# RookieJunChen/FullSubNet-plus

Hardware: AMD Instinct MI355X
Metric: STFT frames/sec (257-bin, 2 s clips), FullSubNet+ forward (higher is better)
Workload: dtype f32

## Files before the change

fullsubnet_plus_amd/csrc/lstm.hip:

```cpp
#include <cstring>

#include "fsnp_common.h"
#include "lstm_common.h"

namespace fsnp {

template <int EX>
__host__ __device__ __forceinline__ int e_frag_index(int e, int k) {
    return ((((k >> 3) * 2) + (k & 1)) * EX + e) * 4 + ((k >> 1) & 3);
}

struct WStream {
    __amdgpu_buffer_rsrc_t rsrc;
    int voff;
};
template <int NT>
__device__ __forceinline__ float4 wload(const WStream& ws, int g, int n) {
    const auto v = __builtin_amdgcn_raw_buffer_load_b128(ws.rsrc, ws.voff, (g * NT + n) * 1024, 0);
    return __builtin_bit_cast(float4, v);
}

template <int NT, int EX>
__device__ __forceinline__ void mfma_groups(f32x16 (&acc)[NT], float (&accx)[EX > 0 ? EX : 1][NT], float4 (&b)[NT],
                                            const float4* __restrict__ A, const float4* __restrict__ AE, int ngroups,
                                            const WStream& ws, int& gnext, int groups_total) {
    float4 a = A[0];
    float4 ae[EX > 0 ? EX : 1];
#pragma unroll
    for (int e = 0; e < EX; ++e) ae[e] = AE[e];
    for (int g = 0; g < ngroups; ++g) {
        const int gn = (g + 1 < ngroups ? g + 1 : g);
        const float4 an = A[gn * 64];
        float4 aen[EX > 0 ? EX : 1];
#pragma unroll
        for (int e = 0; e < EX; ++e) aen[e] = AE[gn * 2 * EX + e];
        if constexpr (EX == 0) {
#pragma unroll
            for (int n = 0; n < NT; ++n) {
                acc[n] = __builtin_amdgcn_mfma_f32_32x32x2f32(a.x, b[n].x, acc[n], 0, 0, 0);
                acc[n] = __builtin_amdgcn_mfma_f32_32x32x2f32(a.y, b[n].y, acc[n], 0, 0, 0);
                acc[n] = __builtin_amdgcn_mfma_f32_32x32x2f32(a.z, b[n].z, acc[n], 0, 0, 0);
                acc[n] = __builtin_amdgcn_mfma_f32_32x32x2f32(a.w, b[n].w, acc[n], 0, 0, 0);
                b[n] = wload<NT>(ws, gnext, n);
                __builtin_amdgcn_sched_barrier(0);
            }
        } else {
            constexpr int HALF = NT / 2;
#pragma unroll
            for (int hb = 0; hb < NT; hb += HALF) {
#pragma unroll
                for (int n = hb; n < hb + HALF; ++n) {
                    acc[n] = __builtin_amdgcn_mfma_f32_32x32x2f32(a.x, b[n].x, acc[n], 0, 0, 0);
                    acc[n] = __builtin_amdgcn_mfma_f32_32x32x2f32(a.y, b[n].y, acc[n], 0, 0, 0);
                    acc[n] = __builtin_amdgcn_mfma_f32_32x32x2f32(a.z, b[n].z, acc[n], 0, 0, 0);
                    acc[n] = __builtin_amdgcn_mfma_f32_32x32x2f32(a.w, b[n].w, acc[n], 0, 0, 0);
                }
                __builtin_amdgcn_sched_barrier(0);
#pragma unroll
                for (int n = hb; n < hb + HALF; ++n)
#pragma unroll
                    for (int e = 0; e < EX; ++e) {
                        float v = accx[e][n];
                        v = fmaf(ae[e].x, b[n].x, v);
                        v = fmaf(ae[e].y, b[n].y, v);
                        v = fmaf(ae[e].z, b[n].z, v);
                        accx[e][n] = fmaf(ae[e].w, b[n].w, v);
                    }
                __builtin_amdgcn_sched_barrier(0);
#pragma unroll
                for (int n = hb; n < hb + HALF; ++n) b[n] = wload<NT>(ws, gnext, n);
                __builtin_amdgcn_sched_barrier(0);
            }
        }
        gnext = (gnext + 1 == groups_total) ? 0 : gnext + 1;
        a = an;
#pragma unroll
        for (int e = 0; e < EX; ++e) ae[e] = aen[e];
    }
}

__device__ __forceinline__ unsigned short bf16_bits(float v) {
    const unsigned u = __float_as_uint(v);
    return (unsigned short)((u + 0x7FFFu + ((u >> 16) & 1u)) >> 16);
}
__host__ __device__ __forceinline__ int a_frag_index_bf16(int row, int k) {
    return (((k >> 4) * 64) + (((k >> 3) & 1) * 32) + row) * 8 + (k & 7);
}

template <int ST, int UW, int HBLO = 0>
__device__ __forceinline__ void lstm_cell(f32x16 (&acc)[4 * ST], f32x2 (&c)[ST][8], float* __restrict__ Hs, int wave,
                                          int lane, unsigned short* __restrict__ Hb = nullptr) {
#pragma unroll
    for (int s = 0; s < ST; ++s) {
        const int k = wave * UW + s * 32 + (lane & 31);
        const int kbase = (((k >> 3) * 64) + ((k & 1) * 32)) * 4 + ((k >> 1) & 3);
#pragma unroll
        for (int r = 0; r < 16; r += 2) {
            auto rd = [](float v) {
                if constexpr (ST > 1) { float o; asm("v_accvgpr_read_b32 %0, %1" : "=v"(o) : "a"(v)); return o; }
                else return v;
            };
            const f32x2 h = lstm_cell_pair(f32x2{rd(acc[s][r]), rd(acc[s][r + 1])}, f32x2{rd(acc[ST + s][r]), rd(acc[ST + s][r + 1])},
                                           f32x2{rd(acc[2 * ST + s][r]), rd(acc[2 * ST + s][r + 1])},
                                           f32x2{rd(acc[3 * ST + s][r]), rd(acc[3 * ST + s][r + 1])}, c[s][r >> 1]);
            const int row = (r & 3) + 8 * (r >> 2) + 4 * (lane >> 5);
            Hs[kbase + row * 4] = h.x;
            Hs[kbase + (row + 1) * 4] = h.y;
            if (Hb) {
                const unsigned short hx = bf16_bits(h.x), hy = bf16_bits(h.y);
                Hb[a_frag_index_bf16(row, k)] = hx; Hb[a_frag_index_bf16(row + 1, k)] = hy;
                if constexpr (HBLO > 0) {
                    Hb[HBLO + a_frag_index_bf16(row, k)] = bf16_bits(h.x - __uint_as_float((unsigned)hx << 16));
                    Hb[HBLO + a_frag_index_bf16(row + 1, k)] = bf16_bits(h.y - __uint_as_float((unsigned)hy << 16));
                }
            }
        }
    }
}

using bf16x8 = __attribute__((ext_vector_type(8))) __bf16;
template <int NT, int EX, int ALO>
__device__ __forceinline__ void mfma_groups_bf16(f32x16 (&acc)[NT], float (&accx)[EX > 0 ? EX : 1][NT], float4 (&b)[NT],
                                                 const float4* __restrict__ A, const float4* __restrict__ AE, int nsteps,
                                                 const WStream& ws, int& gnext, int groups_total, int lane) {
    float4 a = A[0], al = A[ALO];
    for (int g = 0; g < nsteps; ++g) {
        const float4 an = A[(g + 1 < nsteps ? g + 1 : g) * 64], aln = A[ALO + (g + 1 < nsteps ? g + 1 : g) * 64];
        float4 he[EX > 0 ? EX : 1][2];
        if constexpr (EX > 0) {
            const int kg = 2 * g + (lane >> 5);
#pragma unroll
            for (int e = 0; e < EX; ++e) { he[e][0] = AE[(kg * 2 + 0) * EX + e]; he[e][1] = AE[(kg * 2 + 1) * EX + e]; }
        }
#pragma unroll
        for (int n = 0; n < NT; ++n) {
            if constexpr (EX > 0) {
                const unsigned w0 = __float_as_uint(b[n].x), w1 = __float_as_uint(b[n].y), w2 = __float_as_uint(b[n].z),
                               w3 = __float_as_uint(b[n].w);
#pragma unroll
                for (int e = 0; e < EX; ++e) {
                    float v = accx[e][n];
                    v = fmaf(he[e][0].x, __uint_as_float(w0 << 16), v);
                    v = fmaf(he[e][1].x, __uint_as_float(w0 & 0xFFFF0000u), v);
                    v = fmaf(he[e][0].y, __uint_as_float(w1 << 16), v);
                    v = fmaf(he[e][1].y, __uint_as_float(w1 & 0xFFFF0000u), v);
                    v = fmaf(he[e][0].z, __uint_as_float(w2 << 16), v);
                    v = fmaf(he[e][1].z, __uint_as_float(w2 & 0xFFFF0000u), v);
                    v = fmaf(he[e][0].w, __uint_as_float(w3 << 16), v);
                    accx[e][n] = fmaf(he[e][1].w, __uint_as_float(w3 & 0xFFFF0000u), v);
                }
            }
            acc[n] = __builtin_amdgcn_mfma_f32_32x32x16_bf16(__builtin_bit_cast(bf16x8, a), __builtin_bit_cast(bf16x8, b[n]),
                                                             acc[n], 0, 0, 0);
            if constexpr (ALO > 0)
                acc[n] = __builtin_amdgcn_mfma_f32_32x32x16_bf16(__builtin_bit_cast(bf16x8, al), __builtin_bit_cast(bf16x8, b[n]),
                                                                 acc[n], 0, 0, 0);
            b[n] = wload<NT>(ws, gnext, n);
            __builtin_amdgcn_sched_barrier(0);
        }
        gnext = (gnext + 1 == groups_total) ? 0 : gnext + 1;
        a = an; al = aln;
    }
}

template <int ST, int UW, int EX, int NT>
__device__ __forceinline__ void lstm_cell_extra(float (&accx)[EX > 0 ? EX : 1][NT], float (&cx)[EX > 0 ? EX : 1][ST],
                                                const float* __restrict__ bias, float* __restrict__ He, int wave,
                                                int lane) {
#pragma unroll
    for (int e = 0; e < EX; ++e)
#pragma unroll
        for (int s = 0; s < ST; ++s) {
            float g4[4];
#pragma unroll
            for (int q = 0; q < 4; ++q) {
                const float v = accx[e][q * ST + s];
                g4[q] = v + __shfl_xor(v, 32) + (bias ? bias[(q * ST + s) * 32] : 0.0f);
            }
            const float cn = fast_sigmoid(g4[1]) * cx[e][s] + fast_sigmoid(g4[0]) * fast_tanh(g4[2]);
            cx[e][s] = cn;
            const float h = fast_sigmoid(g4[3]) * fast_tanh(cn);
            if (lane < 32) He[e_frag_index<EX>(e, wave * UW + s * 32 + lane)] = h;
        }
}

template <int HID, int KX, int OUT, int EX, bool PROF, int NW, bool BF>
__global__ __launch_bounds__(64 * NW) __attribute__((amdgpu_waves_per_eu(NW / 4, NW / 4)))
void lstm2_fc_kernel(LstmWeights w, LstmArgs a) {
    static_assert(OUT == 2, "FC lane mapping assumes output_size == 2");
    static_assert(EX >= 0 && EX <= 4, "at most 4 VALU rows per tile (one FC wave per extra row)");
    static_assert(NW % 4 == 0 && NW >= 4, "whole waves per SIMD");
    constexpr int NTHR = 64 * NW;
    constexpr int UW = HID / NW, ST = UW / 32, NT = 4 * ST;
    static_assert(UW % 32 == 0 && UW * NW == HID, "hidden/NW must be a multiple of 32");
    constexpr int KGX = KX / 8, KGH = HID / 8, KG0 = KGX + KGH;
    constexpr int KSB = HID / 16;
    constexpr int KG1 = BF ? KGH + KSB : 2 * KGH, KGT = KG0 + KG1;
    static_assert(KGH % 4 == 0, "FC k-split");
    static_assert(!BF || HID % 16 == 0, "bf16 k-steps");
    constexpr int RT = 32 + EX;
    constexpr int EXA = EX > 0 ? EX : 1;

    extern __shared__ __attribute__((aligned(16))) unsigned char smem_raw[];
    float4* Xs = reinterpret_cast<float4*>(smem_raw);
    float4* H0s = Xs + KGX * 64;
    float4* H1s = H0s + KGH * 64;
    float4* XEs = H1s + KGH * 64;
    float4* HE0s = XEs + KGX * 2 * EX;
    float4* HE1s = HE0s + KGH * 2 * EX;
    float4* Wfc4 = HE1s + KGH * 2 * EX;
    RowDesc* rows_s = reinterpret_cast<RowDesc*>(Wfc4 + OUT * KGH * 2);
    constexpr int BL = BF ? 1 : 2;
    constexpr bool HILO = BF && EX == 0;
    float* Bs = reinterpret_cast<float*>(rows_s + RT);
    float4* H0b = reinterpret_cast<float4*>(Bs + BL * NW * NT * 32);

    const int tid = threadIdx.x;
    const int lane = tid & 63;
    const int wave = __builtin_amdgcn_readfirstlane(tid >> 6);
    const int slot0 = blockIdx.x * RT;
    const int Tp = a.Tp;

    __shared__ unsigned long long clk_s[2];
    if (a.clk != nullptr && tid == 0) {
        clk_s[1] = __builtin_amdgcn_s_memrealtime();
        clk_s[0] = __builtin_amdgcn_s_memtime();
        if (blockIdx.x == 0) { a.clk[0] = clk_s[0]; a.clk[1] = clk_s[1]; a.clk[4] = 0ull; a.clk[5] = 0ull; a.clk[6] = ~0ull; }
    }

    for (int i = tid; i < (KGX + 2 * KGH) * (64 + 2 * EX); i += NTHR) Xs[i] = make_float4(0.f, 0.f, 0.f, 0.f);
    for (int i = tid; i < OUT * KGH * 2; i += NTHR) {
        const int o = i / (KGH * 2), kg = (i >> 1) % KGH, kh = i & 1;
        const float* wr = w.wfc + (size_t)o * HID + kg * 8 + kh;
        Wfc4[i] = make_float4(wr[0], wr[2], wr[4], wr[6]);
    }
    if (tid < RT) rows_s[tid] = a.rows[slot0 + tid];
    for (int i = tid; i < BL * NW * NT * 32; i += NTHR) {
        const int col = i & 31, n = (i >> 5) % NT, wv = (i / (32 * NT)) % NW, layer = BF ? 1 : i / (32 * NT * NW);
        Bs[i] = w.bias[layer * 4 * HID + (n / ST) * HID + wv * UW + (n % ST) * 32 + col];
    }
    __syncthreads();
    if constexpr (BF) {
        if (tid < 32) reinterpret_cast<float*>(Xs)[a_frag_index(tid, w.NIN)] = 1.0f;
        if (EX > 0 && tid < EX) reinterpret_cast<float*>(XEs)[e_frag_index<EXA>(tid, w.NIN)] = 1.0f;
    }

    const bool dense = a.dense != nullptr;
    const float* __restrict__ gbase = dense ? a.dense : a.att_mag;
    const int gstep = dense ? w.NIN : a.FP;
    auto plan = [&](const RowDesc& rd, int j) -> int {
        if (!rd.valid || j >= w.NIN) return -1;
        if (dense) return rd.b * Tp * w.NIN + j;
        return sb_feature_offset(j, rd.f, rd.b * Tp * a.FP, a.F, a.NSBN, a.NFBN, a.fb_rel, a.fb_branch_stride);
    };
    auto row_md = [&](const RowDesc& rd, int slot, NormMD& md, const NormMD*& md_row) {
        md.m = 0.0f; md.d = 1.0f; md_row = nullptr;
        if (dense || !rd.valid) return;
        if (a.md_row != nullptr) md_row = a.md_row + (size_t)slot * Tp;
        else md = a.md_utt[rd.b];
    };
    constexpr int JSTEP = NTHR / 32, NG = (KX + JSTEP - 1) / JSTEP;
    const int grow = tid & 31;
    int goff[NG], xdst[NG];
    NormMD md; const NormMD* md_row;
    {
        const RowDesc rd = rows_s[grow];
#pragma unroll
        for (int i = 0; i < NG; ++i) {
            const int j = (tid >> 5) + JSTEP * i;
            goff[i] = (j < KX && !(BF && j == w.NIN)) ? plan(rd, j) : -2;
            xdst[i] = a_frag_index(grow, j < KX ? j : 0);
        }
        row_md(rd, slot0 + grow, md, md_row);
    }
    int goffx = -1, xdstx = 0;
    NormMD mdx = {0.0f, 1.0f}; const NormMD* mdx_row = nullptr;
    bool havex = EX > 0 && tid < EX * KX;
    if (BF && havex && tid % KX == w.NIN) havex = false;
    if (havex) {
        const int e = tid / KX, j = tid % KX;
        const RowDesc rd = rows_s[32 + e];
        goffx = plan(rd, j);
        xdstx = e_frag_index<EXA>(e, j);
        row_md(rd, slot0 + 32 + e, mdx, mdx_row);
    }

    float* Xf = reinterpret_cast<float*>(Xs);
    float* XEf = reinterpret_cast<float*>(XEs);
    {
        const NormMD m0 = md_row ? md_row[0] : md;
#pragma unroll
        for (int i = 0; i < NG; ++i)
            if (goff[i] != -2) Xf[xdst[i]] = goff[i] >= 0 ? (gbase[goff[i]] - m0.m) / m0.d : 0.0f;
        if (havex) {
            const NormMD mx = mdx_row ? mdx_row[0] : mdx;
            XEf[xdstx] = goffx >= 0 ? (gbase[goffx] - mx.m) / mx.d : 0.0f;
        }
    }

    const float* __restrict__ bias_l0 = BF ? nullptr : Bs + ((0 * NW + wave) * NT) * 32 + (lane & 31);
    const float* __restrict__ bias_l1 = Bs + (((BL - 1) * NW + wave) * NT) * 32 + (lane & 31);
    f32x2 c0[ST][8], c1[ST][8];
    float cx0[EXA][ST], cx1[EXA][ST];
#pragma unroll
    for (int s = 0; s < ST; ++s) {
#pragma unroll
        for (int r = 0; r < 8; ++r) { c0[s][r] = f32x2{0.0f, 0.0f}; c1[s][r] = f32x2{0.0f, 0.0f}; }
#pragma unroll
        for (int e = 0; e < EXA; ++e) { cx0[e][s] = 0.0f; cx1[e][s] = 0.0f; }
    }

    WStream ws;
    ws.rsrc = __builtin_amdgcn_make_buffer_rsrc(const_cast<float*>(w.wpack) + (size_t)wave * KGT * NT * 256, 0,
                                                KGT * NT * 1024, 0x00020000);
    ws.voff = lane * 16;
    float4 breg[NT];
#pragma unroll
    for (int n = 0; n < NT; ++n) breg[n] = wload<NT>(ws, 0, n);
    int gnext = 1;
    auto run_groups = [&](f32x16 (&acc_)[NT], float (&accx_)[EXA][NT], const float4* A_, const float4* AE_, int ng) {
        mfma_groups<NT, EX>(acc_, accx_, breg, A_, AE_, ng, ws, gnext, KGT);
    };

    const int fc_row = (wave & 3) * 8 + (lane & 7);
    const int fc_o = (lane >> 3) & 1;
    const int fc_kp = lane >> 4;
    const RowDesc fc_rd = rows_s[fc_row];
    const RowDesc fcx_rd = (EX > 0 && wave < EX) ? rows_s[32 + (wave < EX ? wave : 0)] : RowDesc{0, 0, 0, 0};

    auto fc_store = [&](int t_of_h) {
      if (wave < 4) {
        constexpr int KGP = KGH / 4;
        float sum = 0.0f;
#pragma unroll 4
        for (int kk = 0; kk < KGP; ++kk) {
            const int kg = fc_kp * KGP + kk;
#pragma unroll
            for (int kh = 0; kh < 2; ++kh) {
                const float4 h4 = H1s[kg * 64 + kh * 32 + fc_row];
                const float4 w4 = Wfc4[(fc_o * KGH + kg) * 2 + kh];
                sum += h4.x * w4.x + h4.y * w4.y + h4.z * w4.z + h4.w * w4.w;
            }
        }
        sum += __shfl_xor(sum, 16);
        sum += __shfl_xor(sum, 32);
        if (fc_kp == 0 && fc_rd.valid && t_of_h >= a.LA)
            a.out[(size_t)fc_rd.out_off + (size_t)fc_o * a.out_stride_o + (t_of_h - a.LA)] = apply_act(sum + w.bfc[fc_o], a.act);
      }
        if (EX > 0 && wave < EX) {
            const int o = lane >> 5;
            const float* he = reinterpret_cast<const float*>(HE1s);
            float sx = 0.0f;
#pragma unroll 4
            for (int i = 0; i < HID / 32; ++i) {
                const int k = (lane & 31) + 32 * i;
                sx += he[e_frag_index<EXA>(wave, k)] * w.wfc[o * HID + k];
            }
#pragma unroll
            for (int m = 16; m > 0; m >>= 1) sx += __shfl_xor(sx, m);
            if ((lane & 31) == 0 && fcx_rd.valid && t_of_h >= a.LA)
                a.out[(size_t)fcx_rd.out_off + (size_t)o * a.out_stride_o + (t_of_h - a.LA)] = apply_act(sx + w.bfc[o], a.act);
        }
    };

    const float4* AEx = XEs + (lane >> 5) * EX;
    const float4* AEh0 = HE0s + (lane >> 5) * EX;
    const float4* AEh1 = HE1s + (lane >> 5) * EX;

    __syncthreads();

    unsigned long long* prof = nullptr;
    int prof_stride = 0;
    if constexpr (PROF) {
        const bool rec = blockIdx.x == 0 && tid == 0;
        prof = a.prof + (rec ? 0 : (size_t)Tp * 8 + (size_t)blockIdx.x * 256 + tid);
        prof_stride = rec ? 8 : 0;
    }
#define FSNP_STAMP(i) do { if constexpr (PROF) prof[t * prof_stride + (prof_stride ? (i) : 0)] = __builtin_amdgcn_s_memtime(); } while (0)

    for (int t = 0; t < Tp; ++t) {
        FSNP_STAMP(0);
        float xr[NG], xrx = 0.0f;
        NormMD mdn = md, mdxn = mdx;
        const bool have_next = (t + 1 < Tp);
        if (have_next) {
            if (md_row) mdn = md_row[t + 1];
#pragma unroll
            for (int i = 0; i < NG; ++i) xr[i] = goff[i] >= 0 ? gbase[goff[i] + (t + 1) * gstep] : 0.0f;
            if (havex) {
                if (mdx_row) mdxn = mdx_row[t + 1];
                xrx = goffx >= 0 ? gbase[goffx + (t + 1) * gstep] : 0.0f;
            }
        }

        f32x16 acc[NT];
        float accx[EXA][NT];
#pragma unroll
        for (int n = 0; n < NT; ++n) {
#pragma unroll
            for (int r = 0; r < 16; ++r) acc[n][r] = BF ? 0.0f : bias_l0[n * 32];
#pragma unroll
            for (int e = 0; e < EXA; ++e) accx[e][n] = 0.0f;
        }
        run_groups(acc, accx, Xs + lane, AEx, KG0);
        FSNP_STAMP(1);
        __syncthreads();
        FSNP_STAMP(2);
        lstm_cell<ST, UW, HILO ? KSB * 64 * 8 : 0>(acc, c0, reinterpret_cast<float*>(H0s), wave, lane, BF ? reinterpret_cast<unsigned short*>(H0b) : nullptr);
        if (EX > 0) lstm_cell_extra<ST, UW, EX, NT>(accx, cx0, bias_l0, reinterpret_cast<float*>(HE0s), wave, lane);
        if (have_next) {
#pragma unroll
            for (int i = 0; i < NG; ++i)
                if (goff[i] != -2) Xf[xdst[i]] = goff[i] >= 0 ? (xr[i] - mdn.m) / mdn.d : 0.0f;
            if (havex) XEf[xdstx] = goffx >= 0 ? (xrx - mdxn.m) / mdxn.d : 0.0f;
        }
        if (t > 0) fc_store(t - 1);
        FSNP_STAMP(3);
        __syncthreads();
        FSNP_STAMP(4);
#pragma unroll
        for (int n = 0; n < NT; ++n) {
#pragma unroll
            for (int r = 0; r < 16; ++r) acc[n][r] = bias_l1[n * 32];
#pragma unroll
            for (int e = 0; e < EXA; ++e) accx[e][n] = 0.0f;
        }
        run_groups(acc, accx, H1s + lane, AEh1, KGH);
        if constexpr (BF) mfma_groups_bf16<NT, EX, HILO ? KSB * 64 : 0>(acc, accx, breg, H0b + lane, HE0s, KSB, ws, gnext, KGT, lane);
        else run_groups(acc, accx, H0s + lane, AEh0, KGH);
        FSNP_STAMP(5);
        __syncthreads();
        FSNP_STAMP(6);
        lstm_cell<ST, UW>(acc, c1, reinterpret_cast<float*>(H1s), wave, lane);
        if (EX > 0) lstm_cell_extra<ST, UW, EX, NT>(accx, cx1, bias_l1, reinterpret_cast<float*>(HE1s), wave, lane);
        FSNP_STAMP(7);
    }
#undef FSNP_STAMP
    __syncthreads();
    fc_store(Tp - 1);
    if (a.clk != nullptr && tid == 0) {
        const unsigned long long m1 = __builtin_amdgcn_s_memtime(), r1 = __builtin_amdgcn_s_memrealtime();
        if (blockIdx.x == 0) { a.clk[2] = m1; a.clk[3] = r1; }
        atomicMax(a.clk + 4, r1 - clk_s[1]);
        atomicMax(a.clk + 5, m1 - clk_s[0]);
        atomicMin(a.clk + 6, r1 - clk_s[1]);
    }
}





template <int EX, int NW, bool BF, int KX, int HID = 384>
static void launch_lstm_ex(const LstmWeights& w, const LstmArgs& a, hipStream_t s) {
    constexpr int OUT = 2;
    constexpr int KGX = KX / 8, KGH = HID / 8, NT = 4 * (HID / NW / 32);
    const size_t smem = (size_t)(KGX + 2 * KGH) * (64 + 2 * EX) * 16 + (size_t)OUT * KGH * 2 * 16 +
                        (32 + EX) * sizeof(RowDesc) + (size_t)(BF ? 1 : 2) * NW * NT * 32 * 4 + (BF ? (size_t)(EX == 0 ? 2 : 1) * (HID / 16) * 64 * 16 : 0);
    LstmWeights wv = w;
    wv.wpack = BF ? (NW == 12 ? w.wpack_bf[1] : w.wpack_bf[0]) : (NW == 12 ? w.wpack12 : w.wpack);
    if constexpr (KX == 40 && HID == 384) {
        if (a.prof != nullptr) {
            auto kern = lstm2_fc_kernel<HID, KX, OUT, EX, true, NW, BF>;
            (void)hipFuncSetAttribute(reinterpret_cast<const void*>(kern), hipFuncAttributeMaxDynamicSharedMemorySize, (int)smem);
            hipLaunchKernelGGL(kern, dim3(a.num_tiles), dim3(64 * NW), smem, s, wv, a);
            return;
        }
    }
    auto kern = lstm2_fc_kernel<HID, KX, OUT, EX, false, NW, BF>;
    static PerDeviceOnce attr_once;
    attr_once.run([&] { (void)hipFuncSetAttribute(reinterpret_cast<const void*>(kern), hipFuncAttributeMaxDynamicSharedMemorySize, (int)smem); });
    hipLaunchKernelGGL(kern, dim3(a.num_tiles), dim3(64 * NW), smem, s, wv, a);
}

template <int NW, bool BF, int KX>
static void launch_lstm_nw(const LstmWeights& w, const LstmArgs& a, hipStream_t s) {
    switch (a.ex) {
        case 0: launch_lstm_ex<0, NW, BF, KX>(w, a, s); break;
        case 1: launch_lstm_ex<1, NW, BF, KX>(w, a, s); break;
        case 2: launch_lstm_ex<2, NW, BF, KX>(w, a, s); break;
        default: launch_lstm_ex<4, NW, BF, KX>(w, a, s); break;
    }
}

void launch_lstm(const LstmWeights& w, const LstmArgs& a, hipStream_t s) {
    if (a.num_tiles <= 0) return;
    const int waves = w.waves != 0 ? w.waves : (a.ex > 0 ? 12 : 4);
    if (w.H == 256) {
        if (w.KX == 64) launch_lstm_ex<0, 4, false, 64, 256>(w, a, s);
        else launch_lstm_ex<0, 4, false, 40, 256>(w, a, s);
        return;
    }
    if (w.KX == 64) {
        if (waves == 12) launch_lstm_nw<12, false, 64>(w, a, s);
        else launch_lstm_nw<4, false, 64>(w, a, s);
    } else if (w.ih_bf16) {
        if (waves == 12) launch_lstm_nw<12, true, 40>(w, a, s);
        else launch_lstm_nw<4, true, 40>(w, a, s);
    } else {
        if (waves == 12) launch_lstm_nw<12, false, 40>(w, a, s);
        else launch_lstm_nw<4, false, 40>(w, a, s);
    }
}

template <int ST, int UW, int HID, bool LOAD>
__device__ __forceinline__ void stream_state_io(f32x2 (&c0)[ST][8], f32x2 (&c1)[ST][8], float* __restrict__ H0, float* __restrict__ H1,
                                                const RowDesc* __restrict__ rows_s, float* __restrict__ state, long slot_stride, int done,
                                                int wave, int lane) {
#pragma unroll
    for (int r = 0; r < 16; ++r) {
        const int row = (r & 3) + 8 * (r >> 2) + 4 * (lane >> 5);
        const RowDesc rd = rows_s[row];
        const bool on = LOAD ? rd.valid > 0 : rd.valid == done;
        float* __restrict__ p = state + (size_t)rd.b * slot_stride + (size_t)rd.f * 4 * HID;
#pragma unroll
        for (int s = 0; s < ST; ++s) {
            const int k = wave * UW + s * 32 + (lane & 31);
            const int hi = (((k >> 3) * 64) + ((k & 1) * 32)) * 4 + ((k >> 1) & 3) + row * 4;
            if constexpr (LOAD) {
                H0[hi] = on ? p[k] : 0.0f;
                c0[s][r >> 1][r & 1] = on ? p[HID + k] : 0.0f;
                H1[hi] = on ? p[2 * HID + k] : 0.0f;
                c1[s][r >> 1][r & 1] = on ? p[3 * HID + k] : 0.0f;
            } else if (on) {
                p[k] = H0[hi];
                p[HID + k] = c0[s][r >> 1][r & 1];
                p[2 * HID + k] = H1[hi];
                p[3 * HID + k] = c1[s][r >> 1][r & 1];
            }
        }
    }
}

template <int HID, int KX>
__global__ __launch_bounds__(256) __attribute__((amdgpu_waves_per_eu(1, 1)))
void lstm2_fc_stream_kernel(LstmWeights w, LstmArgs a) {
    constexpr int NW = 4, NTHR = 256, OUT = 2;
    constexpr int UW = HID / NW, ST = UW / 32, NT = 4 * ST;
    constexpr int KGX = KX / 8, KGH = HID / 8, KG0 = KGX + KGH, KGT = KG0 + 2 * KGH;
    static_assert(UW % 32 == 0 && KGH % 4 == 0, "hidden/4 must be a multiple of 32");

    extern __shared__ __attribute__((aligned(16))) unsigned char smem_raw[];
    float4* Xs = reinterpret_cast<float4*>(smem_raw);
    float4* H0s = Xs + KGX * 64;
    float4* H1s = H0s + KGH * 64;
    float4* Wfc4 = H1s + KGH * 64;
    RowDesc* rows_s = reinterpret_cast<RowDesc*>(Wfc4 + OUT * KGH * 2);
    float* Bs = reinterpret_cast<float*>(rows_s + 32);

    const int tid = threadIdx.x;
    const int lane = tid & 63;
    const int wave = __builtin_amdgcn_readfirstlane(tid >> 6);
    const int slot0 = blockIdx.x * 32;
    const int Tp = a.Tp;

    for (int i = tid; i < (KGX + 2 * KGH) * 64; i += NTHR) Xs[i] = make_float4(0.f, 0.f, 0.f, 0.f);
    for (int i = tid; i < OUT * KGH * 2; i += NTHR) {
        const int o = i / (KGH * 2), kg = (i >> 1) % KGH, kh = i & 1;
        const float* wr = w.wfc + (size_t)o * HID + kg * 8 + kh;
        Wfc4[i] = make_float4(wr[0], wr[2], wr[4], wr[6]);
    }
    if (tid < 32) rows_s[tid] = a.rows[slot0 + tid];
    for (int i = tid; i < 2 * NW * NT * 32; i += NTHR) {
        const int col = i & 31, n = (i >> 5) % NT, wv = (i / (32 * NT)) % NW, layer = i / (32 * NT * NW);
        Bs[i] = w.bias[layer * 4 * HID + (n / ST) * HID + wv * UW + (n % ST) * 32 + col];
    }
    __syncthreads();

    int nsteps = 0, cmin = 1 << 30;
    for (int r = 0; r < 32; ++r) {
        const int v = rows_s[r].valid;
        nsteps = v > nsteps ? v : nsteps;
        if (v > 0) cmin = v < cmin ? v : cmin;
    }
    nsteps = __builtin_amdgcn_readfirstlane(nsteps);
    const bool mixed = __builtin_amdgcn_readfirstlane(cmin < nsteps ? 1 : 0) != 0;
    if (nsteps <= 0) return;

    constexpr int JSTEP = NTHR / 32, NG = (KX + JSTEP - 1) / JSTEP;
    const int grow = tid & 31;
    int goff[NG], xdst[NG];
    const float* __restrict__ gbase = a.att_mag;
    const int gstep = a.FP;
    const NormMD* md_row;
    {
        const RowDesc rd = rows_s[grow];
#pragma unroll
        for (int i = 0; i < NG; ++i) {
            const int j = (tid >> 5) + JSTEP * i;
            goff[i] = j >= KX ? -2 : (rd.valid > 0 && j < w.NIN)
                          ? sb_feature_offset(j, rd.f, rd.b * Tp * a.FP, a.F, a.NSBN, a.NFBN, a.fb_rel, a.fb_branch_stride) : -1;
            xdst[i] = a_frag_index(grow, j < KX ? j : 0);
        }
        md_row = a.md_row + (size_t)(slot0 + grow) * Tp;
    }
    float* Xf = reinterpret_cast<float*>(Xs);
    {
        const NormMD m0 = rows_s[grow].valid > 0 ? md_row[0] : NormMD{0.0f, 1.0f};
#pragma unroll
        for (int i = 0; i < NG; ++i)
            if (goff[i] != -2) Xf[xdst[i]] = goff[i] >= 0 ? (gbase[goff[i]] - m0.m) / m0.d : 0.0f;
    }

    const float* __restrict__ bias_l0 = Bs + ((0 * NW + wave) * NT) * 32 + (lane & 31);
    const float* __restrict__ bias_l1 = Bs + ((1 * NW + wave) * NT) * 32 + (lane & 31);
    f32x2 c0[ST][8], c1[ST][8];
    stream_state_io<ST, UW, HID, true>(c0, c1, reinterpret_cast<float*>(H0s), reinterpret_cast<float*>(H1s), rows_s, a.st_sb, a.st_stride, 0,
                                       wave, lane);

    WStream ws;
    ws.rsrc = __builtin_amdgcn_make_buffer_rsrc(const_cast<float*>(w.wpack) + (size_t)wave * KGT * NT * 256, 0, KGT * NT * 1024, 0x00020000);
    ws.voff = lane * 16;
    float4 breg[NT];
#pragma unroll
    for (int n = 0; n < NT; ++n) breg[n] = wload<NT>(ws, 0, n);
    int gnext = 1;
    float accx[1][NT];
    auto run_groups = [&](f32x16 (&acc_)[NT], const float4* A_, int ng) {
        mfma_groups<NT, 0>(acc_, accx, breg, A_, A_, ng, ws, gnext, KGT);
    };

    const int fc_row = (wave & 3) * 8 + (lane & 7);
    const int fc_o = (lane >> 3) & 1;
    const int fc_kp = lane >> 4;
    const RowDesc fc_rd = rows_s[fc_row];
    auto fc_store = [&](int t_of_h) {
        constexpr int KGP = KGH / 4;
        float sum = 0.0f;
#pragma unroll 4
        for (int kk = 0; kk < KGP; ++kk) {
            const int kg = fc_kp * KGP + kk;
#pragma unroll
            for (int kh = 0; kh < 2; ++kh) {
                const float4 h4 = H1s[kg * 64 + kh * 32 + fc_row];
                const float4 w4 = Wfc4[(fc_o * KGH + kg) * 2 + kh];
                sum += h4.x * w4.x + h4.y * w4.y + h4.z * w4.z + h4.w * w4.w;
            }
        }
        sum += __shfl_xor(sum, 16);
        sum += __shfl_xor(sum, 32);
        if (fc_kp == 0 && t_of_h < fc_rd.valid)
            a.out[(size_t)fc_rd.out_off + (size_t)fc_o * a.out_stride_o + t_of_h] = apply_act(sum + w.bfc[fc_o], a.act);
    };

    __syncthreads();

    for (int t = 0; t < nsteps; ++t) {
        float xr[NG];
        NormMD mdn = {0.0f, 1.0f};
        const bool have_next = (t + 1 < nsteps);
        if (have_next) {
            if (rows_s[grow].valid > 0) mdn = md_row[t + 1];
#pragma unroll
            for (int i = 0; i < NG; ++i) xr[i] = goff[i] >= 0 ? gbase[goff[i] + (t + 1) * gstep] : 0.0f;
        }

        f32x16 acc[NT];
#pragma unroll
        for (int n = 0; n < NT; ++n)
#pragma unroll
            for (int r = 0; r < 16; ++r) acc[n][r] = bias_l0[n * 32];
        run_groups(acc, Xs + lane, KG0);
        __syncthreads();
        lstm_cell<ST, UW>(acc, c0, reinterpret_cast<float*>(H0s), wave, lane);
        if (have_next) {
#pragma unroll
            for (int i = 0; i < NG; ++i)
                if (goff[i] != -2) Xf[xdst[i]] = goff[i] >= 0 ? (xr[i] - mdn.m) / mdn.d : 0.0f;
        }
        if (t > 0) fc_store(t - 1);
        __syncthreads();
#pragma unroll
        for (int n = 0; n < NT; ++n)
#pragma unroll
            for (int r = 0; r < 16; ++r) acc[n][r] = bias_l1[n * 32];
        run_groups(acc, H1s + lane, KGH);
        run_groups(acc, H0s + lane, KGH);
        __syncthreads();
        lstm_cell<ST, UW>(acc, c1, reinterpret_cast<float*>(H1s), wave, lane);
        if (t + 1 == nsteps || mixed)
            stream_state_io<ST, UW, HID, false>(c0, c1, reinterpret_cast<float*>(H0s), reinterpret_cast<float*>(H1s), rows_s, a.st_sb,
                                                a.st_stride, t + 1, wave, lane);
    }
    __syncthreads();
    fc_store(nsteps - 1);
}

template <int HID, int KX>
static void launch_lstm_stream_one(const LstmWeights& w, const LstmArgs& a, hipStream_t s) {
    constexpr int KGX = KX / 8, KGH = HID / 8, NT = 4 * (HID / 4 / 32);
    const size_t smem = (size_t)(KGX + 2 * KGH) * 64 * 16 + (size_t)2 * KGH * 2 * 16 + 32 * sizeof(RowDesc) + (size_t)2 * 4 * NT * 32 * 4;
    auto kern = lstm2_fc_stream_kernel<HID, KX>;
    static PerDeviceOnce attr_once;
    attr_once.run([&] { (void)hipFuncSetAttribute(reinterpret_cast<const void*>(kern), hipFuncAttributeMaxDynamicSharedMemorySize, (int)smem); });
    hipLaunchKernelGGL(kern, dim3(a.num_tiles), dim3(256), smem, s, w, a);
}

bool lstm_stream_available(const LstmWeights& w) {
    return !w.gru && w.OUT == 2 && (w.H == 384 || w.H == 256) && (w.KX == 40 || w.KX == 64) && w.wpack != nullptr;
}

void launch_lstm_stream(const LstmWeights& w, const LstmArgs& a, hipStream_t s) {
    if (a.num_tiles <= 0) return;
    if (w.H == 256) { if (w.KX == 64) launch_lstm_stream_one<256, 64>(w, a, s); else launch_lstm_stream_one<256, 40>(w, a, s); }
    else if (w.KX == 64) launch_lstm_stream_one<384, 64>(w, a, s);
    else launch_lstm_stream_one<384, 40>(w, a, s);
}

LstmPlan plan_lstm_tiles(int num_rows, int num_cus) {
    LstmPlan p{};
    if (num_rows <= 32 * num_cus) {
        p.ex = 0; p.num_tiles = cdiv(num_rows, 32);
    } else {
        const int cand[4] = {0, 1, 2, 4};
        int best_rounds = 1 << 30;
        for (int i = 0; i < 4; ++i) {
            const int rounds = cdiv(cdiv(num_rows, 32 + cand[i]), num_cus);
            if (rounds < best_rounds) { best_rounds = rounds; p.ex = cand[i]; }
        }
        p.num_tiles = best_rounds * num_cus;
    }
    p.rows_per_slot_tile = 32 + p.ex;
    return p;
}

}
```

fullsubnet_plus_amd/csrc/lstm_common.h:

```cpp
#pragma once
#include "fsnp_common.h"

namespace fsnp {

using f32x16 = __attribute__((ext_vector_type(16))) float;

__device__ __forceinline__ float fast_sigmoid(float x) { return __builtin_amdgcn_rcpf(1.0f + __expf(-x)); }
__device__ __forceinline__ float fast_tanh(float x) { return 2.0f * __builtin_amdgcn_rcpf(1.0f + __expf(-2.0f * x)) - 1.0f; }

using f32x2 = __attribute__((ext_vector_type(2))) float;
__device__ __forceinline__ f32x2 exp2_pair(f32x2 x) { return f32x2{__builtin_amdgcn_exp2f(x.x), __builtin_amdgcn_exp2f(x.y)}; }
__device__ __forceinline__ f32x2 rcp_pair(f32x2 x) { return f32x2{__builtin_amdgcn_rcpf(x.x), __builtin_amdgcn_rcpf(x.y)}; }
__device__ __forceinline__ f32x2 min_pair(f32x2 x, float m) { return f32x2{fminf(x.x, m), fminf(x.y, m)}; }
__device__ __forceinline__ f32x2 lstm_cell_pair(f32x2 xi, f32x2 xf, f32x2 xg, f32x2 xo, f32x2& c) {
    constexpr float kS = -1.4426950408889634f, kT = -2.8853900817779268f;
    const f32x2 ei = exp2_pair(xi * kS), ef = exp2_pair(xf * kS), eo = exp2_pair(xo * kS);
    const f32x2 eg = exp2_pair(min_pair(xg * kT, 64.0f));
    const f32x2 igg = (1.0f - eg) * rcp_pair((1.0f + ei) * (1.0f + eg));
    const f32x2 cn = rcp_pair(1.0f + ef) * c + igg;
    c = cn;
    const f32x2 ec = exp2_pair(min_pair(cn * kT, 64.0f));
    return (1.0f - ec) * rcp_pair((1.0f + eo) * (1.0f + ec));
}

__device__ __forceinline__ f32x2 gru_cell_pair(f32x2 ar, f32x2 az, f32x2 anx, f32x2 anh, f32x2 h) {
    constexpr float kS = -1.4426950408889634f, kT = -2.8853900817779268f;
    const f32x2 r = rcp_pair(1.0f + exp2_pair(ar * kS));
    const f32x2 ez = exp2_pair(min_pair(az * kS, 60.0f));
    const f32x2 en = exp2_pair(min_pair((anx + r * anh) * kT, 60.0f));
    const f32x2 num = ez * (1.0f - en) + h * (1.0f + en);
    return num * rcp_pair((1.0f + ez) * (1.0f + en));
}

__device__ __forceinline__ float apply_act(float v, int act) {
    if (act == FSNP_ACT_RELU) return fmaxf(v, 0.0f);
    if (act == FSNP_ACT_RELU6) return fminf(fmaxf(v, 0.0f), 6.0f);
    if (act == FSNP_ACT_TANH) return tanhf(v);
    return v;
}

__host__ __device__ __forceinline__ int a_frag_index(int row, int k) {
    return (((k >> 3) * 64) + ((k & 1) * 32) + row) * 4 + ((k >> 1) & 3);
}


constexpr int kCoopCounterStride = 64;
#define FSNP_COOP_BAR(a, tile, which) ((a).coop_bar_stride ? (a).coop_bar + (size_t)(tile) * (a).coop_bar_stride + (which) * ((a).coop_bar_stride / 2) \
                                                           : ((which) ? (a).coop_bar2 : (a).coop_bar) + (tile))
__host__ __device__ constexpr size_t coop_counter_bytes(int tiles) { return (size_t)tiles * kCoopCounterStride * 4; }
__host__ __device__ constexpr int coop_tile_f4(int HID) { return 5 * (HID / 8) * 64 + 2 * (HID / 8) * 16; }

__host__ __device__ __forceinline__ int xcd_local_tiles(int S, int T, int cus_per_xcd) {
    const int fit = cus_per_xcd / S, need = (T + 7) / 8;
    return fit < need ? fit : need;
}
__host__ __device__ __forceinline__ int xcd_local_blocks_per_xcd(int S, int T, int cus_per_xcd) {
    const int Lx = xcd_local_tiles(S, T, cus_per_xcd);
    const int t_local = T < 8 * Lx ? T : 8 * Lx;
    return Lx * S + ((T - t_local) * S + 7) / 8;
}
__device__ __forceinline__ bool xcd_local_decode(int id, int S, int T, int cus_per_xcd, int& tile, int& cs) {
    const int Lx = xcd_local_tiles(S, T, cus_per_xcd);
    const int t_local = T < 8 * Lx ? T : 8 * Lx;
    const int xcd = id & 7, j = id >> 3;
    if (j < Lx * S) { tile = (j / S) * 8 + xcd; cs = j % S; return tile < t_local; }
    const int q = (j - Lx * S) * 8 + xcd;
    tile = t_local + q / S; cs = q % S;
    return tile < T;
}

constexpr int kSc1 = 16;
__device__ __forceinline__ void xchg_store(float* p, float v) {
    __hip_atomic_store(p, v, __ATOMIC_RELAXED, __HIP_MEMORY_SCOPE_AGENT);
}
__device__ __forceinline__ float xchg_load(const float* p) {
    return __hip_atomic_load(p, __ATOMIC_RELAXED, __HIP_MEMORY_SCOPE_AGENT);
}

constexpr long long kXchgTimeoutTicks = 200000000LL;
__device__ __forceinline__ bool xchg_wait(const unsigned* bar, unsigned target, unsigned* abort_dev, unsigned* err_host) {
    unsigned spins = 0;
    long long t0 = 0;
    while (__hip_atomic_load(bar, __ATOMIC_RELAXED, __HIP_MEMORY_SCOPE_AGENT) < target) {
        __builtin_amdgcn_s_sleep(1);
        if ((++spins & 255u) == 0) {
            if (__hip_atomic_load(abort_dev, __ATOMIC_RELAXED, __HIP_MEMORY_SCOPE_AGENT) != 0) return false;
            const long long now = wall_clock64();
            if (t0 == 0) t0 = now;
            else if (now - t0 > kXchgTimeoutTicks) {
                __hip_atomic_store(abort_dev, 1u, __ATOMIC_RELAXED, __HIP_MEMORY_SCOPE_AGENT);
                __hip_atomic_store(err_host, 1u, __ATOMIC_RELAXED, __HIP_MEMORY_SCOPE_SYSTEM);
                return false;
            }
        }
    }
    return true;
}

__device__ __forceinline__ void chaos_delay(int seed, int t, int phase) {
    if (seed == 0) return;
    unsigned h = (unsigned)seed * 2654435761u ^ (unsigned)blockIdx.x * 40503u ^ (unsigned)t * 2246822519u ^ (unsigned)phase * 3266489917u;
    h ^= h >> 15; h *= 2246822519u; h ^= h >> 13; h *= 3266489917u; h ^= h >> 16;
    int n = 0;
    if ((h & 7u) == 0) n = 1 + (int)((h >> 3) & 7u);
    if ((h & 1023u) == 1u) n = 64;
    for (int i = 0; i < n; ++i) __builtin_amdgcn_s_sleep(127);
}

}
```

Before: 144,300.

## Add zero-start LSTM recurrence path with bias folded into activation exponent

For the f32, 4-wave, no-extra-row configuration, adds a specialized time-step loop. The first MFMA of each gate group now starts from a zero accumulator instead of a bias-initialized one. The bias is pre-scaled by the exp2 constants and applied inside the cell activation via an FMA. The first time step is peeled so the weight stream can wrap past the unused layer-1 recurrent groups. This removes the accumulator bias initialization and some weight streaming in step zero, at the cost of a larger code path that duplicates the loop body.

```diff
diff --git a/fullsubnet_plus_amd/csrc/lstm.hip b/fullsubnet_plus_amd/csrc/lstm.hip
--- a/fullsubnet_plus_amd/csrc/lstm.hip
+++ b/fullsubnet_plus_amd/csrc/lstm.hip
@@ -76,6 +76,42 @@
         a = an;
 #pragma unroll
         for (int e = 0; e < EX; ++e) ae[e] = aen[e];
+    }
+}
+
+template <int NT, bool ZERO>
+__device__ __forceinline__ void mfma_group_zs(f32x16 (&acc)[NT], float4 (&b)[NT], const float4 a, const WStream& ws, int& gnext,
+                                              int wrap_at, int wrap_to) {
+    const f32x16 zero = {0.f, 0.f, 0.f, 0.f, 0.f, 0.f, 0.f, 0.f, 0.f, 0.f, 0.f, 0.f, 0.f, 0.f, 0.f, 0.f};
+#pragma unroll
+    for (int n = 0; n < NT; ++n) {
+        acc[n] = __builtin_amdgcn_mfma_f32_32x32x2f32(a.x, b[n].x, ZERO ? zero : acc[n], 0, 0, 0);
+        acc[n] = __builtin_amdgcn_mfma_f32_32x32x2f32(a.y, b[n].y, acc[n], 0, 0, 0);
+        acc[n] = __builtin_amdgcn_mfma_f32_32x32x2f32(a.z, b[n].z, acc[n], 0, 0, 0);
+        acc[n] = __builtin_amdgcn_mfma_f32_32x32x2f32(a.w, b[n].w, acc[n], 0, 0, 0);
+        b[n] = wload<NT>(ws, gnext, n);
+        __builtin_amdgcn_sched_barrier(0);
+    }
+    gnext = (gnext + 1 == wrap_at) ? wrap_to : gnext + 1;
+}
+template <int NT, bool START>
+__device__ __forceinline__ void mfma_groups_zs(f32x16 (&acc)[NT], float4 (&b)[NT], const float4* __restrict__ A, int g0, int g1,
+                                               const WStream& ws, int& gnext, int wrap_at, int wrap_to) {
+    float4 a = A[g0 * 64];
+    int g = g0;
+    if constexpr (START) {
+        const float4 an = A[(g0 + 1) * 64];
+        __builtin_amdgcn_sched_barrier(0);
+        mfma_group_zs<NT, true>(acc, b, a, ws, gnext, wrap_at, wrap_to);
+        a = an;
+        g = g0 + 1;
+    }
+#pragma nounroll
+    for (; g < g1; ++g) {
+        const float4 an = A[(g + 1) * 64];
+        __builtin_amdgcn_sched_barrier(0);
+        mfma_group_zs<NT, false>(acc, b, a, ws, gnext, wrap_at, wrap_to);
+        a = an;
     }
 }
 
@@ -118,6 +154,27 @@
     }
 }
 
+template <int ST, int UW>
+__device__ __forceinline__ void lstm_cell_biased(f32x16 (&acc)[4 * ST], f32x2 (&c)[ST][8], float* __restrict__ Hs, int wave, int lane,
+                                                 const float (&bk)[4 * ST]) {
+#pragma unroll
+    for (int s = 0; s < ST; ++s) {
+        const int k = wave * UW + s * 32 + (lane & 31);
+        const int kbase = (((k >> 3) * 64) + ((k & 1) * 32)) * 4 + ((k >> 1) & 3);
+        const float bi = bk[s], bf = bk[ST + s], bg = bk[2 * ST + s], bo = bk[3 * ST + s];
+#pragma unroll
+        for (int r = 0; r < 16; r += 2) {
+            auto rd = [](float v) { float o; asm("v_accvgpr_read_b32 %0, %1" : "=v"(o) : "a"(v)); return o; };
+            const f32x2 h = lstm_cell_pair(f32x2{rd(acc[s][r]), rd(acc[s][r + 1])}, f32x2{rd(acc[ST + s][r]), rd(acc[ST + s][r + 1])},
+                                           f32x2{rd(acc[2 * ST + s][r]), rd(acc[2 * ST + s][r + 1])},
+                                           f32x2{rd(acc[3 * ST + s][r]), rd(acc[3 * ST + s][r + 1])}, bi, bf, bg, bo, c[s][r >> 1]);
+            const int row = (r & 3) + 8 * (r >> 2) + 4 * (lane >> 5);
+            Hs[kbase + row * 4] = h.x;
+            Hs[kbase + (row + 1) * 4] = h.y;
+        }
+    }
+}
+
 using bf16x8 = __attribute__((ext_vector_type(8))) __bf16;
 template <int NT, int EX, int ALO>
 __device__ __forceinline__ void mfma_groups_bf16(f32x16 (&acc)[NT], float (&accx)[EX > 0 ? EX : 1][NT], float4 (&b)[NT],
@@ -183,6 +240,8 @@
             if (lane < 32) He[e_frag_index<EX>(e, wave * UW + s * 32 + lane)] = h;
         }
 }
+
+template <bool B> struct BoolTag { static constexpr bool value = B; };
 
 template <int HID, int KX, int OUT, int EX, bool PROF, int NW, bool BF>
 __global__ __launch_bounds__(64 * NW) __attribute__((amdgpu_waves_per_eu(NW / 4, NW / 4)))
@@ -200,6 +259,7 @@
     static_assert(!BF || HID % 16 == 0, "bf16 k-steps");
     constexpr int RT = 32 + EX;
     constexpr int EXA = EX > 0 ? EX : 1;
+    constexpr bool ZS = NW == 4 && EX == 0 && !BF;
 
     extern __shared__ __attribute__((aligned(16))) unsigned char smem_raw[];
     float4* Xs = reinterpret_cast<float4*>(smem_raw);
@@ -237,7 +297,9 @@
     if (tid < RT) rows_s[tid] = a.rows[slot0 + tid];
     for (int i = tid; i < BL * NW * NT * 32; i += NTHR) {
         const int col = i & 31, n = (i >> 5) % NT, wv = (i / (32 * NT)) % NW, layer = BF ? 1 : i / (32 * NT * NW);
-        Bs[i] = w.bias[layer * 4 * HID + (n / ST) * HID + wv * UW + (n % ST) * 32 + col];
+        const float bv = w.bias[layer * 4 * HID + (n / ST) * HID + wv * UW + (n % ST) * 32 + col];
+        if constexpr (ZS) Bs[i] = bv * (n / ST == 2 ? kLstmExpT : kLstmExpS);
+        else Bs[i] = bv;
     }
     __syncthreads();
     if constexpr (BF) {
@@ -378,6 +440,54 @@
     }
 #define FSNP_STAMP(i) do { if constexpr (PROF) prof[t * prof_stride + (prof_stride ? (i) : 0)] = __builtin_amdgcn_s_memtime(); } while (0)
 
+    if constexpr (ZS) {
+        auto step = [&](const int t, auto first_tag) __attribute__((always_inline)) {
+            constexpr bool FIRST = decltype(first_tag)::value;
+            FSNP_STAMP(0);
+            float xr[NG];
+            NormMD mdn = md;
+            const bool have_next = (t + 1 < Tp);
+            if (have_next) {
+                if (md_row) mdn = md_row[t + 1];
+#pragma unroll
+                for (int i = 0; i < NG; ++i) xr[i] = goff[i] >= 0 ? gbase[goff[i] + (t + 1) * gstep] : 0.0f;
+            }
+            f32x16 acc[NT];
+            constexpr int wrap_at = FIRST ? KGX : KGT, wrap_to = FIRST ? KG0 + KGH : 0;
+            float bk[NT];
+            mfma_groups_zs<NT, true>(acc, breg, Xs + lane, 0, FIRST ? KGX : KG0, ws, gnext, wrap_at, wrap_to);
+#pragma unroll
+            for (int n = 0; n < NT; ++n) bk[n] = bias_l0[n * 32];
+            FSNP_STAMP(1);
+            __syncthreads();
+            FSNP_STAMP(2);
+            lstm_cell_biased<ST, UW>(acc, c0, reinterpret_cast<float*>(H0s), wave, lane, bk);
+            if (have_next) {
+#pragma unroll
+                for (int i = 0; i < NG; ++i)
+                    if (goff[i] != -2) Xf[xdst[i]] = goff[i] >= 0 ? (xr[i] - mdn.m) / mdn.d : 0.0f;
+            }
+            if constexpr (!FIRST) fc_store(t - 1);
+            FSNP_STAMP(3);
+            __syncthreads();
+            FSNP_STAMP(4);
+            if constexpr (FIRST) {
+                mfma_groups_zs<NT, true>(acc, breg, H0s + lane, 0, KGH, ws, gnext, KGT, 0);
+            } else {
+                mfma_groups_zs<NT, true>(acc, breg, H1s + lane, 0, KGH, ws, gnext, KGT, 0);
+                mfma_groups_zs<NT, false>(acc, breg, H0s + lane, 0, KGH, ws, gnext, KGT, 0);
+            }
+#pragma unroll
+            for (int n = 0; n < NT; ++n) bk[n] = bias_l1[n * 32];
+            FSNP_STAMP(5);
+            __syncthreads();
+            FSNP_STAMP(6);
+            lstm_cell_biased<ST, UW>(acc, c1, reinterpret_cast<float*>(H1s), wave, lane, bk);
+            FSNP_STAMP(7);
+        };
+        if (Tp > 0) step(0, BoolTag<true>{});
+        for (int t = 1; t < Tp; ++t) step(t, BoolTag<false>{});
+    } else {
     for (int t = 0; t < Tp; ++t) {
         FSNP_STAMP(0);
         float xr[NG], xrx = 0.0f;
@@ -434,6 +544,7 @@
         lstm_cell<ST, UW>(acc, c1, reinterpret_cast<float*>(H1s), wave, lane);
         if (EX > 0) lstm_cell_extra<ST, UW, EX, NT>(accx, cx1, bias_l1, reinterpret_cast<float*>(HE1s), wave, lane);
         FSNP_STAMP(7);
+    }
     }
 #undef FSNP_STAMP
     __syncthreads();
diff --git a/fullsubnet_plus_amd/csrc/lstm_common.h b/fullsubnet_plus_amd/csrc/lstm_common.h
--- a/fullsubnet_plus_amd/csrc/lstm_common.h
+++ b/fullsubnet_plus_amd/csrc/lstm_common.h
@@ -16,6 +16,19 @@
     constexpr float kS = -1.4426950408889634f, kT = -2.8853900817779268f;
     const f32x2 ei = exp2_pair(xi * kS), ef = exp2_pair(xf * kS), eo = exp2_pair(xo * kS);
     const f32x2 eg = exp2_pair(min_pair(xg * kT, 64.0f));
+    const f32x2 igg = (1.0f - eg) * rcp_pair((1.0f + ei) * (1.0f + eg));
+    const f32x2 cn = rcp_pair(1.0f + ef) * c + igg;
+    c = cn;
+    const f32x2 ec = exp2_pair(min_pair(cn * kT, 64.0f));
+    return (1.0f - ec) * rcp_pair((1.0f + eo) * (1.0f + ec));
+}
+
+constexpr float kLstmExpS = -1.4426950408889634f, kLstmExpT = -2.8853900817779268f;
+__device__ __forceinline__ f32x2 fma_pair(f32x2 x, float k, float b) { return __builtin_elementwise_fma(x, f32x2{k, k}, f32x2{b, b}); }
+__device__ __forceinline__ f32x2 lstm_cell_pair(f32x2 xi, f32x2 xf, f32x2 xg, f32x2 xo, float bi, float bf, float bg, float bo, f32x2& c) {
+    constexpr float kS = kLstmExpS, kT = kLstmExpT;
+    const f32x2 ei = exp2_pair(fma_pair(xi, kS, bi)), ef = exp2_pair(fma_pair(xf, kS, bf)), eo = exp2_pair(fma_pair(xo, kS, bo));
+    const f32x2 eg = exp2_pair(min_pair(fma_pair(xg, kT, bg), 64.0f));
     const f32x2 igg = (1.0f - eg) * rcp_pair((1.0f + ei) * (1.0f + eg));
     const f32x2 cn = rcp_pair(1.0f + ef) * c + igg;
     c = cn;
```

New measurement: 144,700 (median of 6 runs). Within noise of the previous version (+0.3%).
